# invictus717/MetaTransformer

Measured on AMD Instinct MI355X. Metric: encoder samples/sec at B=256,N=197,C=768 (Base), higher is better.
Workload: dtype bf16; 1 GPU; BASELINE config 2: Meta-Transformer-Base forward+backward+AdamW, tokens [256,197,768] bf16 per GPU, 12L/768d/12h, fp32 master weights, random init N(0,0.02); mode=train, per_gpu_batch=256, global_batch=256, parallelism=single

## Files before the change

### metatransformer_amd/csrc/gemm.hip

```cpp
#include "gemm_common.h"
#include <string.h>
#include <algorithm>
#include <atomic>

namespace {

constexpr int BM = 128;
constexpr int BN = 128;
constexpr int ROWB = 128;
constexpr int TILE_BYTES = BM * ROWB;
constexpr int NT = 256;

__device__ __forceinline__ int lds_off(int row, int byteoff) {
    const int chunk = byteoff >> 4;
    return row * ROWB + (((chunk ^ ((row >> 1) & 7)) << 4) | (byteoff & 15));
}

struct Stage { u32x4 v[4]; };

template <typename T>
__device__ __forceinline__ void load_nt(Stage& s, const T* __restrict__ S, int64_t ld, int64_t nrows, int64_t K,
                                        int64_t r0, int64_t k0, int tid) {
    constexpr int E = 16 / sizeof(T);
#pragma unroll
// ... 479 lines not shown
                pl.ws_bytes = (size_t)pl.tail_split * (size_t)pl.tail_rows * (size_t)d->N * sizeof(float);
            }
        }
        if (pl.tail_rows == 0 && tiles * kSmallSplitDen <= SLOTS && nk >= (small_nt ? 64 : 16) &&
            (!small_nt || tiles <= 96 || nk >= kSmallSplitLongK)) {
            int s = (int)(SLOTS / tiles);
            while (s > 1 && nk / s < 8) --s;
            if (s >= 2) {
                pl.tail_rows = d->M;
                pl.tail_ksteps = (nk + s - 1) / s;
                pl.tail_split = (nk + pl.tail_ksteps - 1) / pl.tail_ksteps;
                pl.ws_bytes = (size_t)pl.tail_split * (size_t)d->M * (size_t)d->N * sizeof(float);
            }
        }
    }
    return pl;
}

int fill_params(const me_gemm_desc* d, GemmParams& p) {
    ME_CHECK_ARG(d != nullptr, "me_gemm: null descriptor");
    ME_CHECK_ARG(d->op == ME_GEMM_NT || d->op == ME_GEMM_TN, "me_gemm: bad op %d", d->op);
    ME_CHECK_ARG(me_dtype_ok(d->ab_dtype) && (me_out_dtype_ok(d->c_dtype) || d->c_dtype == ME_BF16X2), "me_gemm: bad dtype");
    if (me_is_planes(d->c_dtype))
        ME_CHECK_ARG(d->op == ME_GEMM_NT && d->beta == 0.0f && d->ldc >= (d->c_dtype == ME_BF16X3 ? 3 : 2) * d->N && d->out_group_rows == 0 && !d->colsum_a,
                     "me_gemm: ME_BF16X3 / ME_BF16X2 output: NT, beta = 0, ldc >= 3 N / 2 N, plain rows");
    ME_CHECK_ARG(d->a_wrap_k == 0 || (d->op == ME_GEMM_NT && d->ab_dtype == ME_BF16 && d->a_wrap_k > 0 && d->a_wrap_k % 128 == 0 && d->a_wrap_k < d->K &&
                                      d->K - d->a_wrap_k <= d->a_wrap_k && d->lda >= d->a_wrap_k),
                 "me_gemm: a_wrap_k: NT, bf16, a multiple of 128 with K / 2 <= a_wrap_k < K, lda >= a_wrap_k");
    ME_CHECK_ARG(d->M > 0 && d->N > 0 && d->K > 0, "me_gemm: empty problem M=%lld N=%lld K=%lld",
                 (long long)d->M, (long long)d->N, (long long)d->K);
    ME_CHECK_ARG(d->A && d->B && d->C, "me_gemm: null operand");
    const int E = d->ab_dtype == ME_BF16 ? 8 : 4;
    ME_CHECK_ARG(d->N % 4 == 0, "me_gemm: N=%lld must be a multiple of 4", (long long)d->N);
    ME_CHECK_ARG(d->ldc % 4 == 0, "me_gemm: ldc must be a multiple of 4");
    if (d->op == ME_GEMM_NT) {
        ME_CHECK_ARG(d->K % E == 0 && d->lda % E == 0 && d->ldb % E == 0,
                     "me_gemm(NT): K, lda, ldb must be multiples of %d elements (16 bytes)", E);
    } else {
        ME_CHECK_ARG(d->M % E == 0 && d->N % E == 0 && d->lda % E == 0 && d->ldb % E == 0,
                     "me_gemm(TN): M, N, lda, ldb must be multiples of %d elements (16 bytes)", E);
    }
    ME_CHECK_ARG(((uintptr_t)d->A | (uintptr_t)d->B | (uintptr_t)d->C) % 16 == 0, "me_gemm: operands must be 16-byte aligned");
    ME_CHECK_ARG(d->act == ME_ACT_NONE || d->act == ME_ACT_GELU, "me_gemm: bad act");
    ME_CHECK_ARG((d->flags & ~(ME_GEMM_SAVE_GELU_GRAD | ME_GEMM_AUX_IS_FACTOR)) == 0, "me_gemm: unknown flags");
    ME_CHECK_ARG(!(d->flags & ME_GEMM_SAVE_GELU_GRAD) || (d->act == ME_ACT_GELU && d->preact), "me_gemm: ME_GEMM_SAVE_GELU_GRAD needs act = GELU and preact");
    ME_CHECK_ARG(!(d->flags & ME_GEMM_AUX_IS_FACTOR) || d->aux, "me_gemm: ME_GEMM_AUX_IS_FACTOR needs aux");
    if (d->preact) ME_CHECK_ARG((me_dtype_ok(d->preact_dtype) && d->ldpre % 4 == 0) ||
                                (d->preact_dtype == ME_GG8 && d->flags == ME_GEMM_SAVE_GELU_GRAD && d->ldpre % 8 == 0 && (uintptr_t)d->preact % 8 == 0), "me_gemm: bad preact");
    if (d->aux) ME_CHECK_ARG((me_dtype_ok(d->aux_dtype) && d->ldaux % 4 == 0) ||
                             (d->aux_dtype == ME_GG8 && d->flags == ME_GEMM_AUX_IS_FACTOR && d->ldaux % 8 == 0 && (uintptr_t)d->aux % 8 == 0), "me_gemm: bad aux");
    if (d->residual) ME_CHECK_ARG(me_dtype_ok(d->res_dtype) && d->ldres % 4 == 0, "me_gemm: bad residual");
    p.A = d->A; p.B = d->B; p.C = d->C;
    p.M = d->M; p.N = d->N; p.K = d->K; p.lda = d->lda; p.ldb = d->ldb; p.ldc = d->ldc;
    p.c_dtype = d->c_dtype; p.act = d->act; p.alpha = d->alpha; p.beta = d->beta;
    p.bias = d->bias; p.colscale = d->colscale;
    p.preact = d->preact; p.ldpre = d->ldpre; p.preact_dtype = d->preact_dtype;
    p.flags = d->flags;
    p.aux = d->aux; p.ldaux = d->ldaux; p.aux_dtype = d->aux_dtype;
    p.residual = d->residual; p.ldres = d->ldres; p.res_dtype = d->res_dtype;
    p.res_row_mod = d->res_row_mod; p.out_group_rows = d->out_group_rows;
    p.out_group_stride = d->out_group_stride; p.out_row_offset = d->out_row_offset;
    p.split_k = 1; p.ksteps_per_split = 0;
    p.colsum_ws = nullptr;
    ME_CHECK_ARG((d->row_affine == nullptr && d->row_parts == nullptr) == (d->col_shift == nullptr), "me_gemm: row_affine (or row_parts) and col_shift go together");
    ME_CHECK_ARG(!d->row_affine || d->op == ME_GEMM_NT, "me_gemm: row_affine (folded LayerNorm) is defined for ME_GEMM_NT");
    p.row_affine = d->row_affine; p.col_shift = d->col_shift;
    p.row_nparts = 0; p.row_eps = 0.0f;
    p.sk_wgs = 0; p.sk_upt = 0; p.sk_levels = 0; p.sk_l1 = 0;
    p.a_wrap_kt = (int)(d->a_wrap_k / 64);
    if (d->row_parts) {
        ME_CHECK_ARG(!d->row_affine && d->col_shift && d->op == ME_GEMM_NT, "me_gemm: row_parts replaces row_affine (NT, with col_shift)");
        ME_CHECK_ARG(d->row_nparts >= 1 && d->row_nparts <= 4 && (int64_t)d->row_nparts * ME_STATS_GROUP == d->K && d->row_eps >= 0.0f,
                     "me_gemm: row_parts: row_nparts = K / 256, 1 .. 4 (see me_gemm_takes_row_parts)");
        ME_CHECK_ARG((uintptr_t)d->row_parts % 8 == 0, "me_gemm: row_parts must be 8-byte aligned");
        p.row_affine = d->row_parts; p.row_nparts = d->row_nparts; p.row_eps = d->row_eps;
    }
    ME_CHECK_ARG(!d->row_stats || (d->op == ME_GEMM_NT && d->residual && (uintptr_t)d->row_stats % 8 == 0),
                 "me_gemm: row_stats goes with ME_GEMM_NT and a residual operand (8-byte aligned)");
    p.row_stats = d->row_stats;
    p.g3_full_tiles = 0; p.g3_split = 0; p.g3_ktp = 0; p.g3_slabs = nullptr; p.slab_stride = 0; p.g3_tickets = nullptr; p.g3_half = 0;
    if (d->colsum_a) ME_CHECK_ARG(d->op == ME_GEMM_TN, "me_gemm: colsum_a is defined for ME_GEMM_TN only");
    p.tiles_m = (int)((d->M + BM - 1) / BM);
    p.tiles_n = (int)((d->N + BN - 1) / BN);
    ME_CHECK_ARG((int64_t)p.tiles_m * p.tiles_n < (1ll << 31), "me_gemm: too many tiles");
    return ME_OK;
}

struct GemmRoute {
    GemmParams p;
    GemmPlan pl;
    G3Form form;
    bool colsum_a = false;
    bool a_wrap = false;
    bool gg8 = false;
    bool row_parts = false;
    bool row_stats_kernel = false, row_stats = false;
};

int route_gemm(const me_gemm_desc* d, GemmRoute& r, bool allow_sk = true) {
    GemmParams& p = r.p;
    const int rc = fill_params(d, p);
    if (rc) return rc;
    const GemmPlan& pl = r.pl = plan_gemm(d, p, allow_sk);
    if (pl.family != GEMM_G128) {
        p.tiles_m = (int)((d->M + pl.bm - 1) / pl.bm);
        p.tiles_n = (int)((d->N + pl.bn - 1) / pl.bn);
    }
    r.colsum_a = d->op == ME_GEMM_TN && ((pl.family == GEMM_G2B && pl.split_k > 1) || pl.family == GEMM_G3);
    if (pl.family != GEMM_G3 || d->op != ME_GEMM_NT) return ME_OK;
    const int cus = g3_cu_count();
    r.form = g3_form(p, cus);
    r.a_wrap = r.form.kernel == G3_ONE_TILE_WRAP;
    r.gg8 = pl.tail_rows == 0 && r.form.kernel == G3_RESIDENT && r.form.pre == G3_PRE_GG8;
    GemmParams pu = p;
    pu.a_wrap_kt = 0;
    const G3Form fu = g3_form(pu, cus);
    const bool resident = pl.tail_rows == 0 && fu.kernel == G3_RESIDENT;
    r.row_parts = resident && fu.pre == G3_PRE_ROW_PARTS && p.M * 8 * 16 < (1ll << 31);
    r.row_stats_kernel = resident && fu.repi == 2;
    r.row_stats = r.row_stats_kernel && p.res_dtype == ME_BF16 && p.N % 256 == 0 && p.M * 8 < (1ll << 31);
    return ME_OK;
}

GemmParams tail_rows_of(const GemmParams& p, int64_t m1) {
    GemmParams pt = p;
    pt.M = p.M - m1;
    pt.C = reinterpret_cast<char*>(p.C) + (size_t)m1 * p.ldc * me_dtype_size(p.c_dtype);
    if (p.preact) pt.preact = reinterpret_cast<char*>(p.preact) + (size_t)m1 * p.ldpre * me_dtype_size(p.preact_dtype);
    if (p.aux) pt.aux = reinterpret_cast<const char*>(p.aux) + (size_t)m1 * p.ldaux * me_dtype_size(p.aux_dtype);
    if (p.residual) pt.residual = reinterpret_cast<const char*>(p.residual) + (size_t)m1 * p.ldres * me_dtype_size(p.res_dtype);
    if (p.row_affine) pt.row_affine = p.row_affine + 2 * m1;
    return pt;
}

int gemm_impl(const me_gemm_desc* d, hipStream_t stream, int* plan_out, GemmTnLaunch tn_launch = nullptr, const void* tn_ctx = nullptr) {
    GemmRoute r;
    int rc = route_gemm(d, r, tn_launch == nullptr);
    if (rc) return rc;
    GemmParams& p = r.p;
    const GemmPlan& pl = r.pl;
    if (tn_launch && !(pl.family == GEMM_G3 && d->op == ME_GEMM_TN)) return ME_ERR_UNSUPPORTED;
    const bool have_ws = pl.ws_bytes && d->workspace && (size_t)d->workspace_bytes >= pl.ws_bytes;
    float* const ws = reinterpret_cast<float*>(d->workspace);
    {
        const int parts = pl.split_k > 1 ? pl.split_k : (pl.tail_rows > 0 ? pl.tail_split : 1);
        *plan_out = (pl.family & 15) | ((have_ws && parts > 1) ? 16 : 0) | (pl.sk_wgs ? 32 : 0) | ((have_ws ? parts : 1) << 8);
    }
    if (d->colsum_a)
        ME_CHECK_ARG(r.colsum_a && have_ws, "me_gemm: colsum_a needs the split-K wgrad kernel and its workspace (see me_gemm_fuses_colsum)");
    if (d->row_stats)
        ME_CHECK_ARG(d->a_wrap_k ? pl.family == GEMM_G3 && d->op == ME_GEMM_NT && pl.tail_rows == 0 : r.row_stats_kernel,
                     "me_gemm: row_stats is not available for this problem (see me_gemm_emits_row_stats)");
    if (d->a_wrap_k)
        ME_CHECK_ARG(r.a_wrap, "me_gemm: a_wrap_k is not available for this problem (see me_gemm_takes_a_wrap)");
    if (d->row_parts)
        ME_CHECK_ARG(r.row_parts, "me_gemm: row_parts is not available for this problem (see me_gemm_takes_row_parts)");
    if ((d->preact && d->preact_dtype == ME_GG8) || (d->aux && d->aux_dtype == ME_GG8))
        ME_CHECK_ARG(r.gg8, "me_gemm: ME_GG8 is not available for this problem (see me_gemm_takes_gg8)");

    if (pl.family == GEMM_G3 && d->op == ME_GEMM_TN) {
        ME_CHECK_ARG(have_ws, "me_gemm(TN, g3): workspace of me_gemm_workspace_bytes() required");
        GemmParams ps = p;
        ps.C = ws;
        ps.split_k = pl.split_k;
        ps.ksteps_per_split = pl.ksteps_per_split;
        ps.slab_stride = g3_tn_slab_stride(d->M, d->N);
// ... 128 lines not shown
```

### metatransformer_amd/csrc/gemm3.hip

```cpp
#include "gemm3_core.h"

namespace {
constexpr int G3_ROWOP_AHEAD = 4;
constexpr int G3_ROWOP_AHEAD_HALF = 4;
constexpr int G3_ROWOP_AHEAD_STATS = 4;

template <int EPI, bool WRAP = false>
__global__ __launch_bounds__(512) __attribute__((amdgpu_waves_per_eu(2, 2))) void gemm_g3_kernel(const GemmParams p) {
    extern __shared__ __attribute__((aligned(16))) char smem[];
    const int tid = threadIdx.x, lane = tid & 63;
    const int wave = __builtin_amdgcn_readfirstlane(tid >> 6);
    const int wr = wave >> 2;

    const int nwg = gridDim.x, bid = blockIdx.x;
    const int xcd = bid & 7, slot = bid >> 3;
    const int F = p.g3_full_tiles;
    const int nf = (F >> 3) + (xcd < (F & 7) ? 1 : 0);
    const int base_f = xcd * (F >> 3) + (xcd < (F & 7) ? xcd : (F & 7));
    int tile, part = -1;
    if (slot < nf) {
        tile = base_f + slot;
    } else {
        const int base_all = xcd * (nwg >> 3) + (xcd < (nwg & 7) ? xcd : (nwg & 7));
        const int tid_ = base_all - base_f + (slot - nf);
        const int tq = __builtin_amdgcn_readfirstlane(tid_ / p.g3_split);
        tile = F + tq;
        part = tid_ - tq * p.g3_split;
    }
    const int tm = __builtin_amdgcn_readfirstlane(tile / p.tiles_n), tn = tile - tm * p.tiles_n;
    const int64_t m0 = (int64_t)tm * G3_BM, n0 = (int64_t)tn * G3_BN;

    G3State s;
    g3_init_lane(s, p, smem, wave, lane);
    g3_zero(s);
    const G3Src src = g3_make_src(p, tm, tn);

    const int nkt = (int)(p.K / G3_BK);
    int kt0 = 0, kt1 = nkt;
    if (part >= 0) {
        kt0 = part * p.g3_ktp;
        kt1 = kt0 + p.g3_ktp < nkt ? kt0 + p.g3_ktp : nkt;
    }
    s.wrap_kt = WRAP ? p.a_wrap_kt : 0;
    g3_issue<0, WRAP>(s, src, 0, kt0); g3_issue<1, WRAP>(s, src, 0, kt0); g3_issue<2, WRAP>(s, src, 0, kt0); g3_issue<3, WRAP>(s, src, 0, kt0);
    g3_issue<0, WRAP>(s, src, 1, kt0 + 1); g3_issue<1, WRAP>(s, src, 1, kt0 + 1); g3_issue<2, WRAP>(s, src, 1, kt0 + 1);
    asm volatile("s_waitcnt vmcnt(6)" ::: "memory");
    __builtin_amdgcn_s_barrier();
    if (wr == 1) __builtin_amdgcn_s_barrier();

    const G3Src null = g3_null_src(p);
    for (int kt = kt0; kt < kt1 - 2; kt += 2) {
        g3_ktile<0, false, 0, false, 0, WRAP>(s, src, kt + 1, src, kt + 2);
        g3_ktile<1, false, 0, false, 0, WRAP>(s, src, kt + 2, src, kt + 3);
    }
    g3_ktile<0, false, 0, false, 0, WRAP>(s, src, kt1 - 1, null, 0);
    g3_ktile<1, false, 0, false, 0, WRAP>(s, null, 0, null, 0);
    asm volatile("s_waitcnt vmcnt(0)" ::: "memory");
    if (wr == 0) __builtin_amdgcn_s_barrier();
    if (part >= 0) {
        const int64_t row0 = (int64_t)(F / p.tiles_n) * G3_BM;
        g3_epilogue<5>(p, s, m0, n0, lane, p.g3_slabs + (int64_t)part * (p.M - row0) * p.N, row0);
        return;
    }
    g3_epilogue<EPI>(p, s, m0, n0, lane);
}

__device__ __forceinline__ int g3_lane_now() {
    unsigned z = 0;
    asm volatile("" : "+v"(z));
    return (int)__builtin_amdgcn_mbcnt_hi(~0u, __builtin_amdgcn_mbcnt_lo(~0u, z));
}
__device__ __forceinline__ unsigned g3r_draw(unsigned* ctr) {
    unsigned old, zero = 0, one = 1;
    unsigned long long saved;
    asm volatile("s_mov_b64 %1, exec\n\ts_mov_b64 exec, 1\n\tglobal_atomic_add %0, %2, %3, %4 sc0\n\ts_mov_b64 exec, %1"
                 : "=&v"(old), "=&s"(saved)
                 : "v"(zero), "v"(one), "s"(ctr)
                 : "memory");
    return old;
}
__device__ __forceinline__ void g3r_publish(unsigned drawn, unsigned* ctr, int nx, uint32_t lds_tick) {
    const unsigned t = __builtin_amdgcn_readfirstlane(drawn);
    if (t == (unsigned)(nx - 1)) {
        unsigned zero = 0;
        unsigned long long saved;
        asm volatile("s_mov_b64 %0, exec\n\ts_mov_b64 exec, 1\n\tglobal_store_dword %1, %1, %2\n\ts_mov_b64 exec, %0"
                     : "=&s"(saved) : "v"(zero), "s"(ctr) : "memory");
    }
    asm volatile("ds_write_b32 %0, %1" ::"v"(lds_tick), "v"(t) : "memory");
}
struct G3Bias { f32x4 v[4]; };
__device__ __forceinline__ G3Bias g3r_bias(const __amdgpu_buffer_rsrc_t brs, int tn, int wave, int lane) {
    G3Bias b;
    (void)lane;
    lane = g3_lane_now();
    const int col = tn * G3_BN + (wave & 3) * 64 + 4 * (lane >> 4);
#pragma unroll
    for (int nt = 0; nt < 4; ++nt)
        b.v[nt] = __builtin_bit_cast(f32x4, __builtin_amdgcn_raw_buffer_load_b128(brs, (col + nt * 16) * 4, 0, 0));
    return b;
}
__device__ __forceinline__ void g3r_set_binit(G3State& s, const G3Bias& b, bool zero) {
    const f32x4 z = {0.f, 0.f, 0.f, 0.f};
#pragma unroll
    for (int j = 0; j < 4; ++j) s.binit[j] = zero ? z : b.v[j];
    asm volatile("" ::"v"(s.binit[0]), "v"(s.binit[1]), "v"(s.binit[2]), "v"(s.binit[3]));
}

__device__ __forceinline__ void g3r_rows8(f32x4& x0, f32x4& x1, f32x4& y0, f32x4& y1) {
#pragma unroll
    for (int e = 0; e < 4; ++e) {
        const unsigned a0 = __float_as_uint(x0[e]), a1 = __float_as_uint(x1[e]), b0 = __float_as_uint(y0[e]), b1 = __float_as_uint(y1[e]);
// ... 259 lines not shown
            if (STATS) {
                unpack(pk, v0, v1);
                unsigned pu = __float_as_uint(v0[0]);
                pu = __builtin_amdgcn_update_dpp(pu, pu, 0x128, 0xf, 0xc, false);
                pu = __builtin_amdgcn_permlane16_swap(pu, pu, false, false)[0];
                pu = __builtin_amdgcn_permlane32_swap(pu, pu, false, false)[0];
                const float P = __uint_as_float(pu);
                const f32x4 d0 = v0 - P, d1 = v1 - P;
                const f32x4 sd = d0 + d1, qd = d0 * d0 + d1 * d1;
                st_s[h] = (sd[0] + sd[1]) + (sd[2] + sd[3]);
                st_q[h] = (qd[0] + qd[1]) + (qd[2] + qd[3]);
                st_p[h] = P;
            }
            __builtin_amdgcn_raw_buffer_store_b128(g3r_lanes(pk, to_mem), crs, (int)(coff + (2 * mt + h) * cstep), 0, EPI == 2 ? G3_POL_C_RES : G3_POL_C);
        }
        if (STATS) {
            auto ror8 = [](float x) { return x + __uint_as_float(__builtin_amdgcn_update_dpp(0u, __float_as_uint(x), 0x128, 0xf, 0xf, true)); };
            const bool b3 = (lane >> 3) & 1, b4 = (lane >> 4) & 1, b5 = (lane >> 5) & 1;
            const float a_s0 = ror8(st_s[0]), a_s1 = ror8(st_s[1]), a_q0 = ror8(st_q[0]), a_q1 = ror8(st_q[1]);
            st_a[mt & 1][0] = b3 ? a_s1 : a_s0;
            st_a[mt & 1][1] = b3 ? a_q1 : a_q0;
            st_a[mt & 1][2] = b3 ? st_p[1] : st_p[0];
            if (mt & 1) {
                auto fold16 = [](float x, float y) {
                    const auto sw = __builtin_amdgcn_permlane16_swap(__float_as_uint(x), __float_as_uint(y), false, false);
                    return __uint_as_float(sw[0]) + __uint_as_float(sw[1]);
                };
                const int k = (mt >> 1) & 1;
                st_b[k][0] = fold16(st_a[0][0], st_a[1][0]);
                st_b[k][1] = fold16(st_a[0][1], st_a[1][1]);
                st_b[k][2] = b4 ? st_a[1][2] : st_a[0][2];
                if ((mt & 3) == 3) {
                    auto fold32 = [](float x, float y) {
                        const auto sw = __builtin_amdgcn_permlane32_swap(__float_as_uint(x), __float_as_uint(y), false, false);
                        return __uint_as_float(sw[0]) + __uint_as_float(sw[1]);
                    };
                    const float S = fold32(st_b[0][0], st_b[1][0]), Q = fold32(st_b[0][1], st_b[1][1]);
                    const float P = b5 ? st_b[1][2] : st_b[0][2];
                    const float ds = S * (1.0f / 64.0f);
                    const u32x2 out = {__float_as_uint(P + ds), __float_as_uint(Q - S * ds)};
                    const int srow = wr * WROWS + 16 * (4 * (mt >> 2) + 2 * (int)b5 + (int)b4) + 8 * (int)b3 + (lane & 7);
                    asm volatile("ds_write_b64 %0, %1" ::"v"(lds_stats + (uint32_t)(srow * 32 + wc * 8)), "v"(out) : "memory");
                }
            }
        }
    }
    if (STATS) {
        asm volatile("s_waitcnt lgkmcnt(0)" ::: "memory");
        __builtin_amdgcn_s_barrier();
        const int t = s.wave * 64 + lane, lr = t >> 1, h = t & 1;
        u32x4 raw;
        asm volatile("ds_read_b128 %0, %1\n\ts_waitcnt lgkmcnt(0)" : "=v"(raw) : "v"(lds_stats + (uint32_t)(lr * 32 + h * 16)) : "memory");
        const float ma = __uint_as_float(raw[0]), qa = __uint_as_float(raw[1]), mb = __uint_as_float(raw[2]), qb = __uint_as_float(raw[3]);
        const float d1 = mb - ma;
        const float m1 = (ma + mb) * 0.5f, q1 = (qa + qb) + d1 * d1 * 32.0f;
        auto swap1 = [](float x) { return __uint_as_float(__builtin_amdgcn_update_dpp(0u, __float_as_uint(x), 0xB1, 0xf, 0xf, true)); };
        const float mo = swap1(m1), qo = swap1(q1);
        const float d2 = mo - m1;
        const u32x2 tot = {__float_as_uint((m1 + mo) * 0.5f), __float_as_uint((q1 + qo) + d2 * d2 * 64.0f)};
        __builtin_amdgcn_raw_buffer_store_b64(tot, srs, h == 0 ? lr * 8 : (int)0x80000000u, 0, 0);
    }
    if (LNP) {
        __builtin_amdgcn_sched_barrier(0);
        g3r_parts_fold(p, lnp, s.wave, lds_tick + 64 + (uint32_t)(par ^ 1) * 2048);
        __builtin_amdgcn_sched_barrier(0);
    }
    if (HALF) {
        constexpr int PAD = (SAVE ? 16 : 8) + ((EPI == 2 || EPI == 6) ? 4 : EPI == 3 ? 8 : 0) ;
        const u32x4 z = {0u, 0u, 0u, 0u};
        const __amdgpu_buffer_rsrc_t none = __builtin_amdgcn_make_buffer_rsrc(p.C, 0, 0, 0x00020000);
#pragma unroll
        for (int i = 0; i < PAD; ++i) __builtin_amdgcn_raw_buffer_store_b128(z, none, 0, 0, 0);
    }
    __builtin_amdgcn_sched_barrier(0);
    g3r_set_binit(s, nb, next_zero);
    if (ctr && s.wave == 0) {
        asm volatile("s_waitcnt vmcnt(%0)" ::"n"(2 + 4 + 16 + (SAVE ? 16 : 0) + ((EPI == 2 || EPI == 3 || EPI == 6) ? (HALF ? 8 : 16) : 0)) : "memory");
        g3r_publish(drawn, ctr, nx, lds_tick);
    }
}

template <int EPI, int PRE> constexpr int g3r_seam() { return (PRE == 1 || PRE == 2 || (PRE == 6 && EPI == 1)) ? 32 : EPI >= 2 ? 20 : 16; }

template <int EPI, int PRE, bool HI = false>
__global__ __launch_bounds__(512) __attribute__((amdgpu_waves_per_eu(2, 2))) void gemm_g3r_kernel(const GemmParams p) {
    constexpr int SEAM = g3r_seam<EPI, PRE>();
    extern __shared__ __attribute__((aligned(16))) char smem[];
    const int tid = threadIdx.x, lane = tid & 63;
    const int wave = __builtin_amdgcn_readfirstlane(tid >> 6);
    const int wr = wave >> 2;

    const int bid = blockIdx.x, xcd = bid & 7, c = bid >> 3, G8 = gridDim.x >> 3;
    const int tiles = p.tiles_m * p.tiles_n, F = p.g3_full_tiles;
    const int nwork = F + (tiles - F) * 2;
    const int nf = (F >> 3) + (xcd < (F & 7) ? 1 : 0);
    const int nx = (nwork >> 3) + (xcd < (nwork & 7) ? 1 : 0);
    const int base_f = xcd * (F >> 3) + (xcd < (F & 7) ? xcd : (F & 7));
    const int base_all = xcd * (nwork >> 3) + (xcd < (nwork & 7) ? xcd : (nwork & 7));
    const int nkt = (int)(p.K / G3_BK);
    auto decode = [&](int slot, int& tile, int& part, int& kt0, int& kt1) {
        part = -1; kt0 = 0; kt1 = nkt;
        if (slot < nf) {
            tile = base_f + slot;
        } else {
            const int pi = base_all - base_f + (slot - nf);
            tile = F + (pi >> 1);
            part = pi & 1;
        }
    };
    auto src_of = [&](int tile, int part, int& tm, int& tn) {
        tm = __builtin_amdgcn_readfirstlane(tile / p.tiles_n);
        tn = tile - tm * p.tiles_n;
        return part >= 0 ? g3_make_src_half(p, tm, tn, part, wr) : g3_make_src(p, tm, tn);
    };
    const bool dyn = p.g3_tickets != nullptr;
    unsigned* const ctr = dyn ? p.g3_tickets + xcd * 16 : nullptr;
    const uint32_t lds_tick = (uint32_t)(uintptr_t)smem + G3_LDS;
    int slot = c;
    if (slot >= nx) return;

    G3State s;
    g3_init_lane(s, p, smem, wave, lane);
    const G3Src null = g3_null_src(p);
    const __amdgpu_buffer_rsrc_t brs = __builtin_amdgcn_make_buffer_rsrc(const_cast<float*>(p.bias), 0, p.bias ? (int)(p.N * 4) : 0, 0x00020000);
    auto prime = [&]() {
        const u32x4 z = {0u, 0u, 0u, 0u};
#pragma unroll
        for (int i = 0; i < SEAM; ++i) __builtin_amdgcn_raw_buffer_store_b128(z, null.a, 0, 0, 0);
    };

    unsigned drawn0 = 0;
    if (dyn && wave == 0) drawn0 = g3r_draw(ctr);

    int tile, part, kt0, kt1, tm, tn;
    decode(slot, tile, part, kt0, kt1);
    G3Src cur = src_of(tile, part, tm, tn);
    g3_issue<0>(s, cur, 0, kt0); g3_issue<1>(s, cur, 0, kt0); g3_issue<2>(s, cur, 0, kt0); g3_issue<3>(s, cur, 0, kt0);
    g3_issue<0>(s, cur, 1, kt0 + 1); g3_issue<1>(s, cur, 1, kt0 + 1); g3_issue<2>(s, cur, 1, kt0 + 1); g3_issue<3>(s, cur, 1, kt0 + 1);
    {
        const G3Bias b0 = g3r_bias(brs, tn, wave, lane);
        g3r_set_binit(s, b0, PRE == 3 || PRE == 5);
    }
    if (PRE == 5) {
        const int64_t m00 = (int64_t)tm * G3_BM + (part >= 0 ? part * 128 : 0);
        int64_t r0 = p.M - m00;
        r0 = r0 < (part >= 0 ? 128 : 256) ? r0 : (part >= 0 ? 128 : 256);
        const G3Parts q0 = g3r_parts_load(p, m00, r0 > 0 ? (int)r0 : 0, wave);
        g3r_parts_fold(p, q0, wave, lds_tick + 64);
    }
    asm volatile("s_waitcnt vmcnt(0)" ::: "memory");
    if (dyn && wave == 0) g3r_publish(drawn0, ctr, nx, lds_tick);
    prime();
    __builtin_amdgcn_s_barrier();
    if (wr == 1) __builtin_amdgcn_s_barrier();

    int item_par = 0;
    while (true) {
        int nslot = 0, ntile = tile, npart = -1, nkt0 = 0, nkt1 = 2, ntm = 0, ntn = 0;
        bool has_next = false;
        G3Src nxt = null;
        auto resolve_next = [&](int ns) {
            nslot = ns;
            has_next = ns < nx;
            if (has_next) {
                decode(nslot, ntile, npart, nkt0, nkt1);
                nxt = src_of(ntile, npart, ntm, ntn);
            }
        };
        if (!dyn) resolve_next(slot + G8);
        const int np = (kt1 - kt0) >> 1;
        auto run_item = [&](auto half_tag) {
            constexpr bool HALF = decltype(half_tag)::value;
            {
                G3Src sb = cur;
                int kb = kt0 + 2, kc = kt0 + 3;
                if (np == 1) { sb = nxt; kb = nkt0; kc = nkt0 + 1; }
                g3_ktile<0, false, SEAM, HALF>(s, cur, 0, sb, kb);
                g3_ktile<1, false, 0, HALF, HALF ? SEAM : 0>(s, sb, kb, sb, kc);
            }
            if (dyn) {
                unsigned t;
                asm volatile("ds_read_b32 %0, %1\n\ts_waitcnt lgkmcnt(0)" : "=v"(t) : "v"(lds_tick) : "memory");
                resolve_next(G8 + (int)__builtin_amdgcn_readfirstlane(t));
            }
            for (int i = 1; i < np; ++i) {
                const int k = kt0 + 2 * i;
                G3Src sb = cur;
                int kb = k + 2, kc = k + 3;
                if (i == np - 1) { sb = nxt; kb = nkt0; kc = nkt0 + 1; }
                g3_ktile<0, false, 0, HALF>(s, cur, k + 1, sb, kb);
                g3_ktile<1, false, 0, HALF>(s, sb, kb, sb, kc);
            }
            if (wr == 0) __builtin_amdgcn_s_barrier();
            int64_t nm0 = 0;
            int nrows = 0;
// ... 128 lines not shown
        g3_issue<0>(s, src, 0, kt0); g3_issue<1>(s, src, 0, kt0); g3_issue<2>(s, src, 0, kt0); g3_issue<3>(s, src, 0, kt0);
        g3_issue<0>(s, src, 1, kt0 + 1); g3_issue<1>(s, src, 1, kt0 + 1); g3_issue<2>(s, src, 1, kt0 + 1);
        asm volatile("s_waitcnt vmcnt(6)" ::: "memory");
        __builtin_amdgcn_s_barrier();
        if (wr == 1) __builtin_amdgcn_s_barrier();
        const bool cs_any = do_cs;
        s.cs[0] = s.cs[1] = 0.f;
        int cs_turn = regular ? tn : (tn + p.tiles_n - ((kt0 >> 1) % p.tiles_n)) % p.tiles_n;
        auto my_turn = [&]() {
            if (!cs_any) return false;
            const bool mine = cs_turn == 0;
            cs_turn = mine ? p.tiles_n - 1 : cs_turn - 1;
            return mine;
        };
        for (int kt = kt0; kt < kt1 - 2; kt += 2) {
            const bool c = my_turn();
            g3_ktile<0, true>(s, src, kt + 1, src, kt + 2, c);
            g3_ktile<1, true>(s, src, kt + 2, src, kt + 3, c);
        }
        {
            const bool c = my_turn();
            g3_ktile<0, true>(s, src, kt1 - 1, null, 0, c);
            g3_ktile<1, true>(s, null, 0, null, 0, c);
        }
        asm volatile("s_waitcnt vmcnt(0)" ::: "memory");
        if (wr == 0) __builtin_amdgcn_s_barrier();
        if (cs_any) {
            float c0 = s.cs[0], c1 = s.cs[1];
            c0 += __shfl_xor(c0, 16, 64); c0 += __shfl_xor(c0, 32, 64);
            c1 += __shfl_xor(c1, 16, 64); c1 += __shfl_xor(c1, 32, 64);
            if (lane < 16) {
                float* row = p.colsum_ws + (int64_t)cs_row * p.M;
                const int wcol = wave & 3;
                const int64_t ma = m0 + wr * 128 + wcol * 16 + lane, mb = ma + 64;
                if (ma < p.M) row[ma] = c0;
                if (mb < p.M) row[mb] = c1;
            }
        }
        g3_epilogue<5>(p, s, m0, n0, g3_lane_now(), reinterpret_cast<float*>(p.C) + (int64_t)part * p.slab_stride, 0);
        u0 = ue;
    }
}


unsigned* g3r_tickets(hipStream_t stream) {
    constexpr int SETS = 64, SET_WORDS = 8 * 16;
    struct Pool {
        unsigned* base = nullptr;
        bool failed = false;
        int next = 0;
        std::map<hipStream_t, int> idx;
    };
    static std::mutex mu;
    static std::map<int, Pool> pools;
    hipStreamCaptureStatus st = hipStreamCaptureStatusNone;
    if (hipStreamIsCapturing(stream, &st) != hipSuccess || st != hipStreamCaptureStatusNone) return nullptr;
    int dev = 0;
    if (hipStreamGetDevice(stream, &dev) != hipSuccess) (void)hipGetDevice(&dev);
    std::lock_guard<std::mutex> lock(mu);
    Pool& P = pools[dev];
    if (!P.base) {
        if (P.failed) return nullptr;
        unsigned* buf = nullptr;
        if (hipMalloc(&buf, (size_t)SETS * SET_WORDS * sizeof(unsigned)) != hipSuccess ||
            hipMemset(buf, 0, (size_t)SETS * SET_WORDS * sizeof(unsigned)) != hipSuccess) {
            P.failed = true;
            return nullptr;
        }
        P.base = buf;
    }
    auto it = P.idx.find(stream);
    if (it == P.idx.end()) {
        if (P.next >= SETS) return nullptr;
        unsigned* set = P.base + (size_t)P.next * SET_WORDS;
        if (hipMemsetAsync(set, 0, SET_WORDS * sizeof(unsigned), stream) != hipSuccess) return nullptr;
        it = P.idx.emplace(stream, P.next++).first;
    }
    return P.base + (size_t)it->second * SET_WORDS;
}

template <int EPI, int PRE> int launch3r(const GemmParams& q0, int G, hipStream_t stream) {
    constexpr bool HI = EPI == 0 || EPI == 2 || EPI == 1;
    constexpr int LDS_BYTES = G3_LDS + 64 + (PRE == 5 ? 4096 : PRE == 4 ? 8192 : 0);
    static OncePerDevice once;
    if (once.need())
        (void)hipFuncSetAttribute(reinterpret_cast<const void*>(&gemm_g3r_kernel<EPI, PRE, HI>), hipFuncAttributeMaxDynamicSharedMemorySize, LDS_BYTES);
    GemmParams q = q0;
    const int tiles = q.tiles_m * q.tiles_n, rem = tiles % G;
    q.g3_full_tiles = tiles; q.g3_split = 1; q.g3_half = 0;
    if (HI && tiles >= G && rem > 0 && 2 * rem <= G && q.K >= 4 * G3_BK) {
        q.g3_full_tiles = tiles - rem;
        q.g3_half = 1;
    }
    q.g3_tickets = q.K >= 4 * G3_BK ? g3r_tickets(stream) : nullptr;
    hipLaunchKernelGGL((gemm_g3r_kernel<EPI, PRE, HI>), dim3((unsigned)G), dim3(512), LDS_BYTES, stream, q);
    ME_CHECK_LAUNCH("me_gemm(g3 resident)");
    return ME_OK;
}

int launch3r_any(int epi, int pre, const GemmParams& q, int G, hipStream_t stream) {
    switch (epi) {
        case 0: return pre == G3_PRE_ROW_PARTS ? launch3r<0, G3_PRE_ROW_PARTS>(q, G, stream) : pre == G3_PRE_ROW_AFFINE ? launch3r<0, G3_PRE_ROW_AFFINE>(q, G, stream) : launch3r<0, G3_PRE_NONE>(q, G, stream);
        case 1: return pre == G3_PRE_GG8 ? launch3r<1, G3_PRE_GG8>(q, G, stream) : pre == G3_PRE_ROW_PARTS ? launch3r<1, G3_PRE_ROW_PARTS>(q, G, stream) :
                       pre == G3_PRE_ROW_AFFINE ? launch3r<1, G3_PRE_ROW_AFFINE>(q, G, stream) : pre == G3_PRE_SAVE_GELU_GRAD ? launch3r<1, G3_PRE_SAVE_GELU_GRAD>(q, G, stream) :
                       pre ? launch3r<1, G3_PRE_SAVE_PREACT>(q, G, stream) : launch3r<1, G3_PRE_NONE>(q, G, stream);
        case 2: return pre == G3_PRE_ROW_STATS ? launch3r<2, G3_PRE_ROW_STATS>(q, G, stream) : launch3r<2, G3_PRE_NONE>(q, G, stream);
        case 3: return launch3r<3, G3_PRE_NONE>(q, G, stream);
        default: return pre == G3_PRE_GG8 ? launch3r<6, G3_PRE_GG8>(q, G, stream) : launch3r<6, G3_PRE_NONE>(q, G, stream);
    }
}

template <int EPI, bool WRAP> int launch3t(const GemmParams& q, int nwg, hipStream_t stream) {
    static OncePerDevice once;
    if (once.need())
        (void)hipFuncSetAttribute(reinterpret_cast<const void*>(&gemm_g3_kernel<EPI, WRAP>), hipFuncAttributeMaxDynamicSharedMemorySize, G3_LDS);
    hipLaunchKernelGGL((gemm_g3_kernel<EPI, WRAP>), dim3((unsigned)nwg), dim3(512), G3_LDS, stream, q);
    ME_CHECK_LAUNCH(WRAP ? "me_gemm(g3, wrapped A)" : "me_gemm(g3)");
    return ME_OK;
}

template <int EPI> int launch3e(const GemmParams& q, const G3Form& f, hipStream_t stream) {
    if constexpr (EPI == 0 || EPI == 4 || EPI == 8)
        if (f.kernel == G3_ONE_TILE_WRAP) return launch3t<EPI, true>(q, f.nwg, stream);
    return launch3t<EPI, false>(q, f.nwg, stream);
}

}

unsigned* me_work_counters(hipStream_t stream) { return g3r_tickets(stream); }

int launch_g3_tn(const GemmParams& p, hipStream_t stream) {
    static OncePerDevice once;
    if (once.need())
        (void)hipFuncSetAttribute(reinterpret_cast<const void*>(&gemm_g3tn_kernel), hipFuncAttributeMaxDynamicSharedMemorySize, G3_LDS);
    const int nwg = p.tiles_m * p.tiles_n * p.split_k;
    hipLaunchKernelGGL(gemm_g3tn_kernel, dim3((unsigned)nwg), dim3(512), G3_LDS, stream, p);
    ME_CHECK_LAUNCH("me_gemm(g3 tn)");
    return ME_OK;
}

int launch_g3_tn_sk(const GemmParams& p, hipStream_t stream) {
    static OncePerDevice once;
    if (once.need())
        (void)hipFuncSetAttribute(reinterpret_cast<const void*>(&gemm_g3tn_sk_kernel), hipFuncAttributeMaxDynamicSharedMemorySize, G3_LDS);
    hipLaunchKernelGGL(gemm_g3tn_sk_kernel, dim3((unsigned)p.sk_wgs), dim3(512), G3_LDS, stream, p);
    ME_CHECK_LAUNCH("me_gemm(g3 tn, balanced partition)");
    return ME_OK;
}

bool g3_tn_supported(const GemmParams& p) {
    return p.M % 8 == 0 && p.N % 8 == 0 && p.lda % 8 == 0 && p.ldb % 8 == 0 && p.K * p.lda * 2 < (1ll << 31) &&
           p.K * p.ldb * 2 < (1ll << 31);
}

bool g3_supported(const GemmParams& p, int op) {
    if (op != ME_GEMM_NT) return false;
    if (p.K % (2 * G3_BK) != 0 || p.N % 8 != 0) return false;
    if (256 * p.lda * 2 >= (1ll << 31) || 256 * p.ldb * 2 >= (1ll << 31)) return false;
    return true;
}

int g3_cu_count() { return device_cus(); }

G3Form g3_form(const GemmParams& p, int cus) {
    G3Form f;
    const int e = pick_epi_ex(p);
    f.epi = (p.colscale && e != 2 && e != 8) || !((e >= 0 && e <= 3) || (e >= 6 && e <= 10)) ? 4 : e;
    const int EPI = f.epi, tiles = p.tiles_m * p.tiles_n;
    const bool split = p.g3_split > 1 && p.g3_slabs != nullptr;
    f.nwg = split ? p.g3_full_tiles + (tiles - p.g3_full_tiles) * p.g3_split : tiles;
    f.G = cus & ~7;
    if (p.a_wrap_kt) {
        f.kernel = (e == 0 || e == 4 || e == 8) ? G3_ONE_TILE_WRAP : G3_UNSUPPORTED;
        return f;
    }
    f.repi = EPI <= 3 ? EPI : -1;
    f.pre = (EPI == 1 && p.preact) ? G3_PRE_SAVE_PREACT : G3_PRE_NONE;
    const bool plain = p.beta == 0.0f && p.out_group_rows == 0 && p.res_row_mod == 0 && !p.colscale && !p.residual;
    if (EPI == 4 && p.row_affine && !p.flags && plain && !p.preact && !p.aux) {
        f.repi = p.act == ME_ACT_GELU ? 1 : 0;
        f.pre = p.row_nparts ? G3_PRE_ROW_PARTS : G3_PRE_ROW_AFFINE;
    }
    if (EPI == 4 && p.flags && !p.row_affine) {
        if (plain && p.flags == ME_GEMM_SAVE_GELU_GRAD && p.act == ME_ACT_GELU && p.preact && !p.aux) { f.repi = 1; f.pre = G3_PRE_SAVE_GELU_GRAD; }
        if (plain && p.flags == ME_GEMM_AUX_IS_FACTOR && p.act == ME_ACT_NONE && p.aux && (p.aux_dtype == ME_BF16 || p.aux_dtype == ME_GG8) && !p.preact) f.repi = 6;
    }
    if (EPI == 6) f.repi = 6;
    if (EPI == 7) { f.repi = 1; f.pre = G3_PRE_SAVE_GELU_GRAD; }
    if (f.repi == 1 && f.pre == G3_PRE_SAVE_GELU_GRAD && p.preact_dtype == ME_GG8) f.pre = G3_PRE_GG8;
    if (f.repi == 6 && p.aux_dtype == ME_GG8) f.pre = G3_PRE_GG8;
    if (EPI == 2 && p.row_stats) f.pre = G3_PRE_ROW_STATS;
    const int64_t ldmax = std::max(std::max(p.ldc, p.preact ? p.ldpre : 0), std::max(p.residual ? p.ldres : 0, p.aux ? p.ldaux : 0));
    const bool bf16_preact = !(f.pre == G3_PRE_SAVE_PREACT || f.pre == G3_PRE_SAVE_GELU_GRAD) || p.preact_dtype == ME_BF16;
    const bool gg8_rows = f.pre != G3_PRE_GG8 || !p.preact || p.ldpre % 8 == 0;
    const bool resident_only = p.row_stats || p.row_nparts || (p.preact && p.preact_dtype == ME_GG8) || (p.aux && p.aux_dtype == ME_GG8);
    if (f.repi >= 0 && !p.colscale && f.G >= 8 && f.nwg >= f.G && !split && p.alpha == 1.0f && p.c_dtype == ME_BF16 && bf16_preact && gg8_rows &&
        256 * ldmax * 2 < (1ll << 31))
        f.kernel = G3_RESIDENT;
    else
        f.kernel = resident_only ? G3_UNSUPPORTED : G3_ONE_TILE;
    return f;
}

int launch_g3(const GemmParams& p, const G3Form& f, hipStream_t stream) {
    if (f.kernel == G3_UNSUPPORTED) {
        me_set_error("me_gemm(g3): no kernel serves this descriptor");
        return ME_ERR_UNSUPPORTED;
    }
    GemmParams q = p;
    if (q.g3_split <= 1 || q.g3_slabs == nullptr) { q.g3_full_tiles = q.tiles_m * q.tiles_n; q.g3_split = 1; q.g3_ktp = 0; q.g3_slabs = nullptr; }
    if (f.kernel == G3_RESIDENT) return launch3r_any(f.repi, f.pre, q, f.G, stream);
    switch (f.epi) {
        case 0: return launch3e<0>(q, f, stream);
        case 1: return launch3e<1>(q, f, stream);
        case 2: return launch3e<2>(q, f, stream);
        case 3: return launch3e<3>(q, f, stream);
        case 6: return launch3e<6>(q, f, stream);
        case 7: return launch3e<7>(q, f, stream);
        case 8: return launch3e<8>(q, f, stream);
        case 9: return launch3e<9>(q, f, stream);
        case 10: return launch3e<10>(q, f, stream);
        default: return launch3e<4>(q, f, stream);
    }
}
```

### metatransformer_amd/csrc/gemm_common.h

```cpp
#pragma once
#include "common.h"
#include "gemm_host.h"

struct GemmParams {
    const void* A; const void* B; void* C;
    int64_t M, N, K, lda, ldb, ldc;
    int c_dtype, act;
    int flags;
    float alpha, beta;
    const float* bias; const float* colscale;
    void* preact; int64_t ldpre; int preact_dtype;
    const void* aux; int64_t ldaux; int aux_dtype;
    const void* residual; int64_t ldres; int res_dtype;
    int64_t res_row_mod, out_group_rows, out_group_stride, out_row_offset;
    int tiles_m, tiles_n;
    int split_k, ksteps_per_split;
    float* colsum_ws;
    int g3_full_tiles, g3_split, g3_ktp;
    float* g3_slabs;
    int g3_half;
    unsigned* g3_tickets;
    int64_t slab_stride;
    const float* row_affine;
    int row_nparts; float row_eps;
    const float* col_shift;
    int sk_wgs, sk_upt, sk_levels, sk_l1;
    int a_wrap_kt;
    float* row_stats;
};


__host__ __device__ static inline int sk_owner(int64_t u, int E, int64_t TUl) { return (int)(((u + 1) * E - 1) / TUl); }
__host__ __device__ static inline int sk_first(int tile, int E, int Ul, int64_t TUl) { return sk_owner((int64_t)tile * Ul, E, TUl); }
__host__ __device__ static inline int sk_left_parts(int tile, int E, int Ul, int64_t TUl) {
    return Ul > 0 ? sk_owner((int64_t)(tile + 1) * Ul - 1, E, TUl) - sk_first(tile, E, Ul, TUl) + 1 : 0;
}
#define ME_SK_PARTS(p, tile) ((p).sk_levels + sk_left_parts((tile), (p).sk_wgs - (p).sk_levels * (p).tiles_m * (p).tiles_n, (p).sk_upt - (p).sk_levels * (p).sk_l1, \
                                                            (int64_t)(p).tiles_m * (p).tiles_n * ((p).sk_upt - (p).sk_levels * (p).sk_l1)))

__device__ __forceinline__ void epilogue_quad(const GemmParams& p, int64_t m, int64_t n, f32x4 v) {
    v *= p.alpha;
    if (p.row_affine) v = v * p.row_affine[2 * m] + *reinterpret_cast<const f32x4*>(p.col_shift + n) * p.row_affine[2 * m + 1];
    if (p.bias) v += *reinterpret_cast<const f32x4*>(p.bias + n);
    if (p.flags & ME_GEMM_SAVE_GELU_GRAD) {
        f32x4 dv;
        gelu_erf_pair4(v, v, dv);
        store4_from_f32(p.preact, p.preact_dtype, m * p.ldpre + n, dv);
    } else {
        if (p.preact) store4_from_f32(p.preact, p.preact_dtype, m * p.ldpre + n, v);
        if (p.act == ME_ACT_GELU) v = gelu_for4(v, p.c_dtype);
    }
    if (p.aux) {
        const f32x4 a = load4_as_f32(p.aux, p.aux_dtype, m * p.ldaux + n);
        v *= (p.flags & ME_GEMM_AUX_IS_FACTOR) ? a : gelu_grad_for4(a, p.c_dtype);
    }
    if (p.colscale) v *= *reinterpret_cast<const f32x4*>(p.colscale + n);
    if (p.residual) {
        const int64_t rr = p.res_row_mod ? (m % p.res_row_mod) : m;
        v += load4_as_f32(p.residual, p.res_dtype, rr * p.ldres + n);
    }
    const int64_t orow = p.out_group_rows
                             ? (m / p.out_group_rows) * p.out_group_stride + (m % p.out_group_rows) + p.out_row_offset
                             : m;
    if (p.c_dtype == ME_BF16X3) {
        store4_split3(reinterpret_cast<uint16_t*>(p.C) + orow * p.ldc, p.N, n, v);
        return;
    }
    if (p.c_dtype == ME_BF16X2) {
        store4_split2(reinterpret_cast<uint16_t*>(p.C) + orow * p.ldc, p.N, n, v);
        return;
    }
    if (p.beta != 0.0f) v += p.beta * load4_as_f32(p.C, p.c_dtype, orow * p.ldc + n);
    store4_from_f32(p.C, p.c_dtype, orow * p.ldc + n, v);
}



__device__ __forceinline__ void epilogue_quad_lin(const GemmParams& p, int64_t m, int64_t n, f32x4 v) {
    v *= p.alpha;
    if (p.bias) v += *reinterpret_cast<const f32x4*>(p.bias + n);
    if (p.colscale) v *= *reinterpret_cast<const f32x4*>(p.colscale + n);
    if (p.residual) {
        const int64_t rr = p.res_row_mod ? (m % p.res_row_mod) : m;
        v += load4_as_f32(p.residual, p.res_dtype, rr * p.ldres + n);
    }
    const int64_t orow = p.out_group_rows
                             ? (m / p.out_group_rows) * p.out_group_stride + (m % p.out_group_rows) + p.out_row_offset
                             : m;
    if (p.c_dtype == ME_BF16X3) {
        store4_split3(reinterpret_cast<uint16_t*>(p.C) + orow * p.ldc, p.N, n, v);
        return;
    }
    if (p.c_dtype == ME_BF16X2) {
        store4_split2(reinterpret_cast<uint16_t*>(p.C) + orow * p.ldc, p.N, n, v);
        return;
    }
    if (p.beta != 0.0f) v += p.beta * load4_as_f32(p.C, p.c_dtype, orow * p.ldc + n);
    store4_from_f32(p.C, p.c_dtype, orow * p.ldc + n, v);
// ... 63 lines not shown
                             : m;
    if (p.c_dtype == ME_BF16X3) {
        uint16_t* row = reinterpret_cast<uint16_t*>(p.C) + orow * p.ldc;
        store4_split3(row, p.N, n, v0);
        store4_split3(row, p.N, n + 4, v1);
        return;
    }
    if (p.c_dtype == ME_BF16X2) {
        uint16_t* row = reinterpret_cast<uint16_t*>(p.C) + orow * p.ldc;
        store4_split2(row, p.N, n, v0);
        store4_split2(row, p.N, n + 4, v1);
        return;
    }
    if (p.beta != 0.0f) {
        f32x4 c0, c1;
        load8_as_f32(p.C, p.c_dtype, orow * p.ldc + n, c0, c1);
        v0 += p.beta * c0; v1 += p.beta * c1;
    }
    store8_from_f32(p.C, p.c_dtype, orow * p.ldc + n, v0, v1);
}

static inline int pick_epi(const GemmParams& p) {
    if (p.split_k > 1) return 5;
    if (me_is_planes(p.c_dtype)) return 4;
    if (p.flags || p.row_affine) return 4;
    if (p.beta != 0.0f || p.out_group_rows != 0 || p.res_row_mod != 0) return 4;
    const int nrow = (p.residual ? 1 : 0) + (p.aux ? 1 : 0);
    if (nrow > 1) return 4;
    if (p.act == ME_ACT_GELU) return (nrow == 0) ? 1 : 4;
    if (p.preact) return 4;
    if (p.residual) return p.res_dtype == ME_BF16 ? 2 : 4;
    if (p.aux) return p.aux_dtype == ME_BF16 ? 3 : 4;
    return 0;
}

static inline int pick_epi_ex(const GemmParams& p) {
    const int e = pick_epi(p);
    if (me_is_planes(p.c_dtype) && p.split_k <= 1 && !p.row_affine && !p.colscale && !p.residual && p.beta == 0.0f && p.out_group_rows == 0 &&
        p.res_row_mod == 0 && p.ldc % 8 == 0 && p.N % 8 == 0) {
        if (p.act == ME_ACT_GELU && !p.aux && (!p.preact ? p.flags == 0 : (p.flags == ME_GEMM_SAVE_GELU_GRAD && p.preact_dtype == ME_F32 && p.ldpre % 4 == 0)))
            return 9;
        if (p.act == ME_ACT_NONE && p.aux && p.aux_dtype == ME_F32 && p.flags == ME_GEMM_AUX_IS_FACTOR && !p.preact && p.ldaux % 4 == 0) return 10;
    }
    if (e == 4 && p.c_dtype == ME_F32 && p.residual && p.res_dtype == ME_F32 && !p.aux && !p.preact && p.act == ME_ACT_NONE && !p.flags &&
        !p.row_affine && p.beta == 0.0f && p.out_group_rows == 0 && p.res_row_mod == 0 && p.split_k <= 1 && p.ldres % 4 == 0)
        return 8;
    if (e != 4 || me_is_planes(p.c_dtype) || p.row_affine || p.colscale || p.residual || p.beta != 0.0f || p.out_group_rows != 0 || p.res_row_mod != 0) return e;
    if (p.flags == ME_GEMM_AUX_IS_FACTOR && p.act == ME_ACT_NONE && p.aux && (p.aux_dtype == ME_BF16 || p.aux_dtype == ME_GG8) && !p.preact) return 6;
    if (p.flags == ME_GEMM_SAVE_GELU_GRAD && p.act == ME_ACT_GELU && p.preact && !p.aux) return 7;
    return e;
}

enum GemmFamily : int {
    GEMM_G128 = 0,
    GEMM_G2B = 2,
    GEMM_G2W = 3,
    GEMM_G3 = 4,
};
int launch_g2b(const GemmParams& p, int op, int bm, int bn, hipStream_t stream);
bool g2b_supported(const GemmParams& p, int op);
bool g3_supported(const GemmParams& p, int op);

enum G3Kernel : int {
    G3_UNSUPPORTED = 0,
    G3_RESIDENT,
    G3_ONE_TILE,
    G3_ONE_TILE_WRAP,
};
enum G3Pre : int {
    G3_PRE_NONE = 0,
    G3_PRE_SAVE_PREACT = 1,
    G3_PRE_SAVE_GELU_GRAD = 2,
    G3_PRE_ROW_AFFINE = 3,
    G3_PRE_ROW_STATS = 4,
    G3_PRE_ROW_PARTS = 5,
    G3_PRE_GG8 = 6,
};
struct G3Form {
    G3Kernel kernel = G3_UNSUPPORTED;
    int epi = 4;
    int repi = -1, pre = G3_PRE_NONE;
    int G = 0;
    int nwg = 0;
};
G3Form g3_form(const GemmParams& p, int cus);
int g3_cu_count();
int launch_g3(const GemmParams& p, const G3Form& f, hipStream_t stream);
int launch_g3_tn(const GemmParams& p, hipStream_t stream);
int launch_g3_tn_sk(const GemmParams& p, hipStream_t stream);
bool g3_tn_supported(const GemmParams& p);
static inline int64_t g3_tn_slab_stride(int64_t M, int64_t N) { return M * N; }
```

Baseline: 8127 samples/s.

## Add grouped serpentine tile walk to g3 GEMM kernels for weight reuse

Introduces a TileWalk mapping that visits output tiles in blocks of rows and column groups, snaking across column groups, instead of plain row-major order. It is enabled for non-split GEMMs whose weight operand is at least 6 MB, and for resident kernels except the residual epilogues. The aim is better L2/LLC reuse of B and A tiles across concurrently running workgroups. In exchange it adds integer division work per tile and a kernarg read, plus extra template instantiations.

Result: no change. 8137 samples/s (median of 6 runs) (+0.1%).

```diff
diff --git a/metatransformer_amd/csrc/gemm.hip b/metatransformer_amd/csrc/gemm.hip
--- a/metatransformer_amd/csrc/gemm.hip
+++ b/metatransformer_amd/csrc/gemm.hip
@@ -585,6 +585,7 @@
     if (d->colsum_a) ME_CHECK_ARG(d->op == ME_GEMM_TN, "me_gemm: colsum_a is defined for ME_GEMM_TN only");
     p.tiles_m = (int)((d->M + BM - 1) / BM);
     p.tiles_n = (int)((d->N + BN - 1) / BN);
+    p.walk = TileWalk{};
     ME_CHECK_ARG((int64_t)p.tiles_m * p.tiles_n < (1ll << 31), "me_gemm: too many tiles");
     return ME_OK;
 }
diff --git a/metatransformer_amd/csrc/gemm3.hip b/metatransformer_amd/csrc/gemm3.hip
--- a/metatransformer_amd/csrc/gemm3.hip
+++ b/metatransformer_amd/csrc/gemm3.hip
@@ -1,9 +1,23 @@
+#include <cassert>
+#include <cstddef>
 #include "gemm3_core.h"
 
 namespace {
 constexpr int G3_ROWOP_AHEAD = 4;
 constexpr int G3_ROWOP_AHEAD_HALF = 4;
 constexpr int G3_ROWOP_AHEAD_STATS = 4;
+
+__device__ __forceinline__ void g3_tile_of(int item, int& tm, int& tn) {
+#if defined(__HIP_DEVICE_COMPILE__)
+    typedef __attribute__((address_space(4))) const TileWalk* WalkPtr;
+    WalkPtr wp = (WalkPtr)((__attribute__((address_space(4))) const char*)__builtin_amdgcn_kernarg_segment_ptr() + offsetof(GemmParams, walk));
+    asm volatile("" : "+s"(wp));
+    const TileWalk w = *wp;
+    tile_walk(w, __builtin_amdgcn_readfirstlane(item), tm, tn);
+#endif
+    tm = __builtin_amdgcn_readfirstlane(tm);
+    tn = __builtin_amdgcn_readfirstlane(tn);
+}
 
 template <int EPI, bool WRAP = false>
 __global__ __launch_bounds__(512) __attribute__((amdgpu_waves_per_eu(2, 2))) void gemm_g3_kernel(const GemmParams p) {
@@ -27,7 +41,8 @@
         tile = F + tq;
         part = tid_ - tq * p.g3_split;
     }
-    const int tm = __builtin_amdgcn_readfirstlane(tile / p.tiles_n), tn = tile - tm * p.tiles_n;
+    int tm, tn;
+    g3_tile_of(tile, tm, tn);
     const int64_t m0 = (int64_t)tm * G3_BM, n0 = (int64_t)tn * G3_BN;
 
     G3State s;
@@ -453,9 +468,12 @@
 
 template <int EPI, int PRE> constexpr int g3r_seam() { return (PRE == 1 || PRE == 2 || (PRE == 6 && EPI == 1)) ? 32 : EPI >= 2 ? 20 : 16; }
 
-template <int EPI, int PRE, bool HI = false>
+constexpr bool g3r_walks(int epi) { return epi != 2 && epi != 3; }
+
+template <int EPI, int PRE, bool HI = false, bool WALK = false>
 __global__ __launch_bounds__(512) __attribute__((amdgpu_waves_per_eu(2, 2))) void gemm_g3r_kernel(const GemmParams p) {
     constexpr int SEAM = g3r_seam<EPI, PRE>();
+    static_assert(!WALK || g3r_walks(EPI), "the residual forms stay row-major");
     extern __shared__ __attribute__((aligned(16))) char smem[];
     const int tid = threadIdx.x, lane = tid & 63;
     const int wave = __builtin_amdgcn_readfirstlane(tid >> 6);
@@ -480,8 +498,12 @@
         }
     };
     auto src_of = [&](int tile, int part, int& tm, int& tn) {
-        tm = __builtin_amdgcn_readfirstlane(tile / p.tiles_n);
-        tn = tile - tm * p.tiles_n;
+        if constexpr (WALK) {
+            g3_tile_of(tile, tm, tn);
+        } else {
+            tm = __builtin_amdgcn_readfirstlane(tile / p.tiles_n);
+            tn = tile - tm * p.tiles_n;
+        }
         return part >= 0 ? g3_make_src_half(p, tm, tn, part, wr) : g3_make_src(p, tm, tn);
     };
     const bool dyn = p.g3_tickets != nullptr;
@@ -776,9 +798,6 @@
 template <int EPI, int PRE> int launch3r(const GemmParams& q0, int G, hipStream_t stream) {
     constexpr bool HI = EPI == 0 || EPI == 2 || EPI == 1;
     constexpr int LDS_BYTES = G3_LDS + 64 + (PRE == 5 ? 4096 : PRE == 4 ? 8192 : 0);
-    static OncePerDevice once;
-    if (once.need())
-        (void)hipFuncSetAttribute(reinterpret_cast<const void*>(&gemm_g3r_kernel<EPI, PRE, HI>), hipFuncAttributeMaxDynamicSharedMemorySize, LDS_BYTES);
     GemmParams q = q0;
     const int tiles = q.tiles_m * q.tiles_n, rem = tiles % G;
     q.g3_full_tiles = tiles; q.g3_split = 1; q.g3_half = 0;
@@ -787,7 +806,19 @@
         q.g3_half = 1;
     }
     q.g3_tickets = q.K >= 4 * G3_BK ? g3r_tickets(stream) : nullptr;
-    hipLaunchKernelGGL((gemm_g3r_kernel<EPI, PRE, HI>), dim3((unsigned)G), dim3(512), LDS_BYTES, stream, q);
+    auto launch = [&](auto walk_tag) {
+        constexpr bool WALK = decltype(walk_tag)::value;
+        static OncePerDevice once;
+        if (once.need())
+            (void)hipFuncSetAttribute(reinterpret_cast<const void*>(&gemm_g3r_kernel<EPI, PRE, HI, WALK>), hipFuncAttributeMaxDynamicSharedMemorySize, LDS_BYTES);
+        hipLaunchKernelGGL((gemm_g3r_kernel<EPI, PRE, HI, WALK>), dim3((unsigned)G), dim3(512), LDS_BYTES, stream, q);
+    };
+    if constexpr (g3r_walks(EPI)) {
+        if (!tile_walk_is_row_major(q.walk)) launch(std::true_type{});
+        else launch(std::false_type{});
+    } else {
+        launch(std::false_type{});
+    }
     ME_CHECK_LAUNCH("me_gemm(g3 resident)");
     return ME_OK;
 }
@@ -856,6 +887,8 @@
 
 int g3_cu_count() { return device_cus(); }
 
+constexpr int64_t kWalkMinWeightBytes = 6ll << 20;
+
 G3Form g3_form(const GemmParams& p, int cus) {
     G3Form f;
     const int e = pick_epi_ex(p);
@@ -864,6 +897,9 @@
     const bool split = p.g3_split > 1 && p.g3_slabs != nullptr;
     f.nwg = split ? p.g3_full_tiles + (tiles - p.g3_full_tiles) * p.g3_split : tiles;
     f.G = cus & ~7;
+    const bool walks = !split && p.N * p.K * 2 >= kWalkMinWeightBytes;
+    f.walk = walks ? tile_walk_plan(p.tiles_m, p.tiles_n) : tile_walk_make(p.tiles_m, p.tiles_n, 0, 0);
+    assert(tile_walk_is_row_major(f.walk) || (p.tiles_n > 4 && !split));
     if (p.a_wrap_kt) {
         f.kernel = (e == 0 || e == 4 || e == 8) ? G3_ONE_TILE_WRAP : G3_UNSUPPORTED;
         return f;
@@ -889,9 +925,10 @@
     const bool gg8_rows = f.pre != G3_PRE_GG8 || !p.preact || p.ldpre % 8 == 0;
     const bool resident_only = p.row_stats || p.row_nparts || (p.preact && p.preact_dtype == ME_GG8) || (p.aux && p.aux_dtype == ME_GG8);
     if (f.repi >= 0 && !p.colscale && f.G >= 8 && f.nwg >= f.G && !split && p.alpha == 1.0f && p.c_dtype == ME_BF16 && bf16_preact && gg8_rows &&
-        256 * ldmax * 2 < (1ll << 31))
+        256 * ldmax * 2 < (1ll << 31)) {
         f.kernel = G3_RESIDENT;
-    else
+        if (!g3r_walks(f.repi)) f.walk = tile_walk_make(p.tiles_m, p.tiles_n, 0, 0);
+    } else
         f.kernel = resident_only ? G3_UNSUPPORTED : G3_ONE_TILE;
     return f;
 }
@@ -902,6 +939,7 @@
         return ME_ERR_UNSUPPORTED;
     }
     GemmParams q = p;
+    q.walk = f.walk;
     if (q.g3_split <= 1 || q.g3_slabs == nullptr) { q.g3_full_tiles = q.tiles_m * q.tiles_n; q.g3_split = 1; q.g3_ktp = 0; q.g3_slabs = nullptr; }
     if (f.kernel == G3_RESIDENT) return launch3r_any(f.repi, f.pre, q, f.G, stream);
     switch (f.epi) {
diff --git a/metatransformer_amd/csrc/gemm_common.h b/metatransformer_amd/csrc/gemm_common.h
--- a/metatransformer_amd/csrc/gemm_common.h
+++ b/metatransformer_amd/csrc/gemm_common.h
@@ -1,6 +1,7 @@
 #pragma once
 #include "common.h"
 #include "gemm_host.h"
+#include "tile_walk.h"
 
 struct GemmParams {
     const void* A; const void* B; void* C;
@@ -14,6 +15,7 @@
     const void* residual; int64_t ldres; int res_dtype;
     int64_t res_row_mod, out_group_rows, out_group_stride, out_row_offset;
     int tiles_m, tiles_n;
+    TileWalk walk;
     int split_k, ksteps_per_split;
     float* colsum_ws;
     int g3_full_tiles, g3_split, g3_ktp;
@@ -243,6 +245,7 @@
     int repi = -1, pre = G3_PRE_NONE;
     int G = 0;
     int nwg = 0;
+    TileWalk walk = {};
 };
 G3Form g3_form(const GemmParams& p, int cus);
 int g3_cu_count();
diff --git a/metatransformer_amd/csrc/tile_walk.h b/metatransformer_amd/csrc/tile_walk.h
--- /dev/null
+++ b/metatransformer_amd/csrc/tile_walk.h
@@ -0,0 +1,52 @@
+#pragma once
+#include <stdint.h>
+
+#if defined(__HIPCC__) || defined(__CUDACC__)
+#define TILE_WALK_HD __host__ __device__
+#else
+#define TILE_WALK_HD
+#endif
+
+struct TileWalk {
+    int tiles_m, tiles_n;
+    int rows, cols;
+    int last_group;
+};
+
+static inline bool tile_walk_is_row_major(const TileWalk& w) { return w.last_group == 0; }
+
+static inline TileWalk tile_walk_make(int tiles_m, int tiles_n, int rows, int cols) {
+    if (tiles_n <= 4 || cols <= 0 || cols >= tiles_n) return TileWalk{tiles_m, tiles_n, 1, tiles_n, 0};
+    if (rows <= 0 || rows > tiles_m) rows = tiles_m;
+    return TileWalk{tiles_m, tiles_n, rows, cols, (tiles_n + cols - 1) / cols - 1};
+}
+
+#ifndef TILE_WALK_ROWS
+#define TILE_WALK_ROWS 8
+#endif
+#ifndef TILE_WALK_COLS
+#define TILE_WALK_COLS 4
+#endif
+static inline TileWalk tile_walk_plan(int tiles_m, int tiles_n) {
+    const int cols = tiles_n % TILE_WALK_COLS == 0 ? TILE_WALK_COLS : tiles_n % 3 == 0 ? 3 : TILE_WALK_COLS;
+    return tile_walk_make(tiles_m, tiles_n, TILE_WALK_ROWS, cols);
+}
+
+TILE_WALK_HD static inline void tile_walk(const TileWalk& w, int item, int& tm, int& tn) {
+    const uint32_t rows = (uint32_t)w.rows, cols = (uint32_t)w.cols, last_group = (uint32_t)w.last_group;
+    const uint32_t cols_last = (uint32_t)w.tiles_n - last_group * cols;
+    const uint32_t blk = (uint32_t)item / (rows * (uint32_t)w.tiles_n);
+    uint32_t rem = (uint32_t)item - blk * (rows * (uint32_t)w.tiles_n);
+    const uint32_t row0 = blk * rows;
+    const uint32_t rb = row0 + rows > (uint32_t)w.tiles_m ? (uint32_t)w.tiles_m - row0 : rows;
+    const uint32_t shift = (blk & 1u) ? rb * (cols - cols_last) : 0u;
+    rem += shift;
+    const uint32_t j = rem / (rb * cols);
+    rem -= j * (rb * cols);
+    if (j == 0) rem -= shift;
+    const uint32_t g = (blk & 1u) ? last_group - j : j;
+    const uint32_t gw = g == last_group ? cols_last : cols;
+    const uint32_t r = rem / gw;
+    tm = (int)(row0 + r);
+    tn = (int)(g * cols + (rem - r * gw));
+}
```
